# MAC-VO/MAC-VO

Measured on AMD Instinct MI355X. Metric: stereo frames/sec at 640x480 (hot path: cost volume + lookup, keypoint selection, covariance, PGO), higher is better.
Workload: dtype f32 via f16x2 (volume: fp32 operands row-scaled by powers of two and split into two fp16 pieces, three products, fp32 accumulate, scales undone exactly) + f32 (lookup/covariance) + f64 (PGO)

## Files before the change

mac-vo_amd/csrc/kp_select.hip:

```cpp
#include "common.h"
#include <math.h>

namespace {

#ifdef MV_KP_PROFILE
__device__ long long g_kp_stamps[16];
#define KP_STAMP(i) do { if (threadIdx.x == 0) g_kp_stamps[i] = wall_clock64(); } while (0)
#else
#define KP_STAMP(i)
#endif

constexpr int TILE_W = 64;
constexpr int TILE_H = 16;
constexpr int MAX_R = 7;
constexpr unsigned CAND_FLAG = 0x80000000u;

struct KpWs {
    unsigned long long* cand_bits;
    unsigned* rec_idx;
    float* rec_q;
    float* rec_d;
    int* counters;
    size_t lane_bytes;

    __device__ __forceinline__ KpWs lane(int l) const {
        const size_t o = (size_t)l * lane_bytes;
        return KpWs{(unsigned long long*)((char*)cand_bits + o), (unsigned*)((char*)rec_idx + o), (float*)((char*)rec_q + o),
                    (float*)((char*)rec_d + o), (int*)((char*)counters + o), lane_bytes};
    }
};

__device__ __forceinline__ float flow_quality(const float* __restrict__ fc, int plane, int idx) {
    const float c0 = fc[idx], c1 = fc[plane + idx], c2 = fc[2 * plane + idx];
    return (c0 + c1) - 2.f * c2;
}

__device__ __forceinline__ float nanmin(float a, float b) { return (a < b || a != a) ? a : b; }

template <bool FUSE>
__global__ __launch_bounds__(256) void kp_nms_kernel(const float* __restrict__ fc, const float* __restrict__ d0,
                                                      const float* __restrict__ d0c, const float* __restrict__ d1,
                                                      const float* __restrict__ d1c,
                                                      const uint8_t* __restrict__ mask_a,
                                                      const uint8_t* __restrict__ mask_b, mvKpSelectParams p,
                                                      KpWs ws_all, int words_per_row, mvEpiArgs ef) {
    MV_CHAIN_KERNEL_PRIO();
    const KpWs ws = ws_all.lane(blockIdx.z);
    {
        const size_t lp = (size_t)blockIdx.z * p.H * p.W;
        if (fc) fc += 3 * lp;
        if (d0) d0 += lp;
        if (d0c) d0c += lp;
        if (d1) d1 += lp;
        if (d1c) d1c += lp;
        if (mask_a) mask_a += lp;
        if (mask_b) mask_b += lp;
        if (FUSE) {
            ef.flow += 4 * lp; ef.logcov += 4 * lp;
            if (ef.disparity) ef.disparity += lp;
            if (ef.disparity_cov) ef.disparity_cov += lp;
            if (ef.depth) ef.depth += lp;
            if (ef.depth_cov) ef.depth_cov += lp;
            if (ef.bad_mask) ef.bad_mask += lp;
            if (ef.match_flow) ef.match_flow += 2 * lp;
            if (ef.match_cov) ef.match_cov += 3 * lp;
        }
    }
    __shared__ float tile[TILE_H + 2 * MAX_R][TILE_W + 2 * MAX_R + 1];
    __shared__ float hmin[TILE_H + 2 * MAX_R][TILE_W + 1];
    __shared__ int wg_count, wg_base;
    const int H = p.H, W = p.W, plane = H * W;
    const int r = p.kernel_size >> 1;
    const int x0 = blockIdx.x * TILE_W, y0 = blockIdx.y * TILE_H;
    const int tx = threadIdx.x, ty = threadIdx.y;
    const int tid = ty * 64 + tx;
    const bool mapping = p.mode == MV_KP_MAPPING;
    if (tid == 0) wg_count = 0;

    if (!mapping) {
        const int tw = TILE_W + 2 * r, th = TILE_H + 2 * r;
        constexpr int NST = ((TILE_W + 2 * MAX_R) * (TILE_H + 2 * MAX_R) + 255) / 256;
        float qv[NST];
#pragma unroll
        for (int i = 0; i < NST; ++i) {
            const int e = i * 256 + tid;
            const int ly = e / tw, lx = e - ly * tw;
            const int gx = x0 + lx - r, gy = y0 + ly - r;
            float q = INFINITY;
            if (e < tw * th && gx >= 0 && gx < W && gy >= 0 && gy < H) {
                const int idx = gy * W + gx;
                if (FUSE) {
                    const float l0 = ef.logcov[2 * plane + idx], l1 = ef.logcov[3 * plane + idx];
                    const float c0 = ef.cov_is_log ? expf(l0 * 2.f) : l0, c1 = ef.cov_is_log ? expf(l1 * 2.f) : l1;
                    q = (c0 + c1) - 2.f * 0.f;
                } else if (p.mode == MV_KP_NODEPTH) {
                    q = flow_quality(fc, plane, idx);
                } else {
                    q = d0c[idx] + d1c[idx];
                    if (fc) q = q * flow_quality(fc, plane, idx);
                }
            }
            qv[i] = q;
        }
#pragma unroll
        for (int i = 0; i < NST; ++i) {
            const int e = i * 256 + tid;
            const int ly = e / tw, lx = e - ly * tw;
            if (e < tw * th) tile[ly][lx] = qv[i];
        }
        __syncthreads();
        for (int e = tid; e < th * TILE_W; e += 256) {
            const int ly = e >> 6, lx = e & 63;
            float m = tile[ly][lx];
            for (int dx = 1; dx <= 2 * r; ++dx) m = nanmin(m, tile[ly][lx + dx]);
            hmin[ly][lx] = m;
        }
    }
    __syncthreads();

    bool nms_px[TILE_H / 4];
    bool cand_px[TILE_H / 4];
    float q_px[TILE_H / 4];
    int my_nms = 0;
#pragma unroll
    for (int it = 0; it < TILE_H / 4; ++it) {
        const int ly = ty * (TILE_H / 4) + it;
        const int gx = x0 + tx, gy = y0 + ly;
        const bool inimg = gx < W && gy < H;
        const int idx = gy * W + gx;
        bool nms = false, cand = false;
        float q = 0.f;
        if (FUSE && inimg) mv_epilogue_pixel(ef, plane, idx);
        if (inimg) {
            const bool border = p.mask_width > 0 && gx >= p.mask_width && gx < W - p.mask_width &&
                                gy >= p.mask_width && gy < H - p.mask_width;
            if (mapping) {
                cand = border && (d0[idx] < p.max_depth) && (d0c[idx] < p.max_depth_cov);
            } else {
                q = tile[ly + r][tx + r];
                float m = hmin[ly][tx];
                for (int dy = 1; dy <= 2 * r; ++dy) m = nanmin(m, hmin[ly + dy][tx]);
                nms = (q == m);
                cand = nms && border;
                if (cand && p.mode == MV_KP_FULL) cand = (d0[idx] < p.max_depth) && (d1[idx] < p.max_depth);
            }
            if (cand && mask_a) cand = mask_a[idx] != 0;
            if (cand && mask_b) cand = mask_b[idx] != 0;
        }
        const unsigned long long cand_word = __ballot(cand);
        if (tx == 0 && gy < H) ws.cand_bits[(size_t)gy * words_per_row + blockIdx.x] = cand_word;
        nms_px[it] = nms;
        cand_px[it] = cand;
        q_px[it] = q;
        my_nms += nms;
    }
    if (mapping) return;

    int my_off = 0;
    if (my_nms) my_off = atomicAdd(&wg_count, my_nms);
    __syncthreads();
#ifdef MV_KP_FAKE_ATOMIC
    if (tid == 0) wg_base = (blockIdx.y * gridDim.x + blockIdx.x) * 16;
#else
    if (tid == 0) wg_base = wg_count ? atomicAdd(&ws.counters[0], wg_count) : 0;
#endif
    __syncthreads();
    int pos = wg_base + my_off;
#pragma unroll
    for (int it = 0; it < TILE_H / 4; ++it) {
        if (nms_px[it]) {
            const int gx = x0 + tx, gy = y0 + ty * (TILE_H / 4) + it;
            const int idx = gy * W + gx;
            ws.rec_idx[pos] = (unsigned)(((gy * words_per_row + blockIdx.x) << 6) | tx) | (cand_px[it] ? CAND_FLAG : 0u);
            if (p.mode == MV_KP_NODEPTH) {
                ws.rec_q[pos] = q_px[it];
            } else {
                ws.rec_q[pos] = fc ? flow_quality(fc, plane, idx) : 0.f;
                ws.rec_d[pos] = d0c[idx];
            }
            ++pos;
        }
    }
}

__device__ __forceinline__ unsigned float_key(float f) {
    if (f != f) return 0xFFFFFFFFu;
    const unsigned u = __float_as_uint(f);
    return (u & 0x80000000u) ? ~u : (u | 0x80000000u);
}
__device__ __forceinline__ float key_float(unsigned k) {
    const unsigned u = (k & 0x80000000u) ? (k & 0x7FFFFFFFu) : ~k;
    return __uint_as_float(u);
}

#ifndef MV_KP_FINISH_THREADS
#define MV_KP_FINISH_THREADS 1024
#endif

constexpr int RANK_CAP = 256;
constexpr unsigned NAN_KEY = 0xFFFFFFFFu;

template <int NT>
__device__ __forceinline__ int block_exclusive_scan(int v, int* wave_tot , int& total) {
    constexpr int NW = NT / 64;
    const int tid = threadIdx.x;
    int incl = v;
#pragma unroll
    for (int o = 1; o < 64; o <<= 1) {
        const int t = __shfl_up(incl, o, 64);
        if ((tid & 63) >= o) incl += t;
    }
    __syncthreads();
    if ((tid & 63) == 63) wave_tot[tid >> 6] = incl;
    __syncthreads();
    int off = 0;
    total = 0;
#pragma unroll
    for (int w = 0; w < NW; ++w) {
        const int t = wave_tot[w];
        if (w < (tid >> 6)) off += t;
        total += t;
    }
    return off + incl - v;
}

template <int NT, bool CACHED, int RPT, typename F>
__device__ __forceinline__ void for_each_key(const float* __restrict__ vals, int n, const unsigned (&keys)[RPT], F&& f) {
    const int tid = threadIdx.x;
    if (CACHED) {
        const int nr = (n + NT - 1) / NT;
#pragma unroll
        for (int r = 0; r < RPT; ++r)
            if (r < nr && r * NT + tid < n) f(keys[r]);
    } else {
        for (int i = tid; i < n; i += NT) f(float_key(vals[i]));
    }
}

struct MedianLds {
    unsigned hist[2048];
    unsigned lst[RANK_CAP];
    unsigned red_lo[16], red_hi[16];
    int red_cnt[16];
    int wave_tot[16];
    int sh[4];
    unsigned res;
};

template <int NT, bool CACHED, int RPT>
__device__ float block_nanmedian(const float* __restrict__ vals, int n, const unsigned (&keys)[RPT], MedianLds& L) {
    constexpr int NW = NT / 64, BPT = 2048 / NT;
    const int tid = threadIdx.x;
    unsigned lo = NAN_KEY, hi = 0u;
    int cnt = 0;
    for_each_key<NT, CACHED, RPT>(vals, n, keys, [&](unsigned k) {
        if (k != NAN_KEY) {
            lo = min(lo, k);
            hi = max(hi, k);
            ++cnt;
        }
    });
#pragma unroll
    for (int o = 32; o > 0; o >>= 1) {
        lo = min(lo, (unsigned)__shfl_xor((int)lo, o, 64));
        hi = max(hi, (unsigned)__shfl_xor((int)hi, o, 64));
        cnt += __shfl_xor(cnt, o, 64);
    }
    __syncthreads();
    if ((tid & 63) == 0) {
        L.red_lo[tid >> 6] = lo;
        L.red_hi[tid >> 6] = hi;
        L.red_cnt[tid >> 6] = cnt;
    }
    __syncthreads();
    cnt = 0;
#pragma unroll
    for (int w = 0; w < NW; ++w) {
        lo = min(lo, L.red_lo[w]);
        hi = max(hi, L.red_hi[w]);
        cnt += L.red_cnt[w];
    }
    if (cnt <= 0) return NAN;
    int k = (cnt - 1) >> 1;
    for (;;) {
        if (lo == hi) return key_float(lo);
        const unsigned span = hi - lo;
        const int s = max(0, 32 - __clz((int)span) - 11);
#pragma unroll
        for (int j = 0; j < BPT; ++j) L.hist[j * NT + tid] = 0;
        if (tid == 0) L.sh[3] = 0;
        __syncthreads();
        for_each_key<NT, CACHED, RPT>(vals, n, keys, [&](unsigned kk) {
            if (kk >= lo && kk <= hi) atomicAdd(&L.hist[(kk - lo) >> s], 1u);
        });
        __syncthreads();
        int c[BPT], sum = 0;
#pragma unroll
        for (int j = 0; j < BPT; ++j) {
            c[j] = (int)L.hist[tid * BPT + j];
            sum += c[j];
        }
        int total;
        const int excl = block_exclusive_scan<NT>(sum, L.wave_tot, total);
        if (excl <= k && k < excl + sum) {
            int before = excl;
#pragma unroll
            for (int j = 0; j < BPT; ++j) {
                if (k >= before && k < before + c[j]) {
                    L.sh[0] = tid * BPT + j;
                    L.sh[1] = c[j];
                    L.sh[2] = k - before;
                }
                before += c[j];
            }
        }
        __syncthreads();
        const unsigned b = (unsigned)L.sh[0];
        const int cb = L.sh[1];
        k = L.sh[2];
        const unsigned nlo = lo + (b << s);
        const unsigned w = s ? ((1u << s) - 1u) : 0u;
        const unsigned nhi = (hi - nlo < w) ? hi : nlo + w;
        if (cb <= RANK_CAP) {
            for_each_key<NT, CACHED, RPT>(vals, n, keys, [&](unsigned kk) {
                if (kk >= nlo && kk <= nhi) L.lst[atomicAdd(&L.sh[3], 1)] = kk;
            });
            __syncthreads();
            for (int i = tid; i < cb; i += NT) {
                const unsigned e = L.lst[i];
                int rank = 0;
                for (int j = 0; j < cb; ++j) {
                    const unsigned o = L.lst[j];
                    rank += (o < e) || (o == e && j < i);
                }
                if (rank == k) L.res = e;
            }
            __syncthreads();
            return key_float(L.res);
        }
        lo = nlo;
        hi = nhi;
        __syncthreads();
    }
}

template <int NT, bool FAST, int RPT, int WPT, bool USE_D>
__device__ __forceinline__ void kp_finish_body(const mvKpSelectParams& p, const KpWs& ws, int has_flow, int words_per_row,
                                               int32_t* __restrict__ out_cand, int32_t* __restrict__ out_count,
                                               float* __restrict__ out_stats, int n_rec, MedianLds& L,
                                               unsigned long long* lds_words) {
    constexpr int RD = USE_D ? RPT : 1;
    const int tid = threadIdx.x;
    const int H = p.H, W = p.W;
    const bool mapping = p.mode == MV_KP_MAPPING;
    const bool use_f = (p.mode == MV_KP_NODEPTH) || (p.mode == MV_KP_FULL && has_flow);
    const bool use_d = USE_D && (p.mode == MV_KP_FULL);
    const int n_words = H * words_per_row;

    unsigned kq[RPT], kd[RD], ridx[RPT];
    unsigned long long wreg[WPT];
    KP_STAMP(0);
    if (FAST) {
        const int cap = H * W;
#pragma unroll
        for (int r = 0; r < RPT; ++r) {
            const int i = min(r * NT + tid, cap - 1);
            ridx[r] = mapping ? 0u : ws.rec_idx[i];
            kq[r] = use_f ? __float_as_uint(ws.rec_q[i]) : 0u;
            if (USE_D) kd[r] = use_d ? __float_as_uint(ws.rec_d[i]) : 0u;
        }
#pragma unroll
        for (int j = 0; j < WPT; ++j) {
            const int w = j * NT + tid;
            wreg[j] = w < n_words ? ws.cand_bits[w] : 0ull;
        }
#pragma unroll
        for (int r = 0; r < RPT; ++r) {
            const bool live = r * NT + tid < n_rec;
            ridx[r] = live ? ridx[r] : 0u;
            kq[r] = live ? float_key(__uint_as_float(kq[r])) : NAN_KEY;
            if (USE_D) kd[r] = live ? float_key(__uint_as_float(kd[r])) : NAN_KEY;
        }
    }

    float med_f = NAN, thr_f = INFINITY, med_d = NAN, thr_d = INFINITY;
    KP_STAMP(1);
    if (use_f) {
        med_f = block_nanmedian<NT, FAST, RPT>(ws.rec_q, n_rec, kq, L);
        const float prod = med_f * 1.5f;
        thr_f = (prod < p.max_match_cov) ? prod : p.max_match_cov;
    }
    if (use_d) {
        med_d = block_nanmedian<NT, FAST, RD>(ws.rec_d, n_rec, kd, L);
        const float prod = med_d * 1.5f;
        thr_d = (prod < p.max_depth_cov) ? prod : p.max_depth_cov;
    }

    KP_STAMP(2);
    const int per = (n_words + NT - 1) / NT;
    unsigned long long cw[WPT];
    if (FAST) {
        constexpr int NPASS = WPT > 5 * 1024 / NT ? 8 : 2;
        constexpr int TPP = NT / NPASS;
        unsigned fail = 0;
        if (!mapping) {
            const int nr = (n_rec + NT - 1) / NT;
#pragma unroll
            for (int r = 0; r < RPT; ++r) {
                if (r < nr && (ridx[r] & CAND_FLAG)) {
                    bool ok = true;
                    if (use_f) ok = key_float(kq[r]) < thr_f;
                    if (USE_D) { if (ok && use_d) ok = key_float(kd[USE_D ? r : 0]) < thr_d; }
                    if (!ok) fail |= 1u << r;
                }
            }
        }
#pragma unroll
        for (int i = 0; i < WPT; ++i) cw[i] = 0ull;
#pragma unroll 1
        for (int h = 0; h < NPASS; ++h) {
            const int wlo = h * TPP * per, whi = min(wlo + TPP * per, n_words);
#pragma unroll
            for (int j = 0; j < WPT; ++j) {
                const int w = j * NT + tid;
                if (w >= wlo && w < whi) lds_words[w - wlo] = wreg[j];
            }
            __syncthreads();
            if (fail) {
#pragma unroll
                for (int r = 0; r < RPT; ++r) {
                    const int w = (int)((ridx[r] & ~CAND_FLAG) >> 6);
                    if (((fail >> r) & 1u) && w >= wlo && w < whi) atomicAnd(&lds_words[w - wlo], ~(1ull << (ridx[r] & 63)));
                }
            }
            __syncthreads();
            if (tid / TPP == h) {
#pragma unroll
                for (int i = 0; i < WPT; ++i) {
                    const int w = tid * per + i;
                    if (i < per && w < whi) cw[i] = lds_words[w - wlo];
                }
            }
            __syncthreads();
        }
    } else if (!mapping) {
        for (int i = tid; i < n_rec; i += NT) {
            const unsigned ri = ws.rec_idx[i];
            if (ri & CAND_FLAG) {
                bool ok = true;
                if (use_f) ok = ws.rec_q[i] < thr_f;
                if (ok && use_d) ok = ws.rec_d[i] < thr_d;
                if (!ok) atomicAnd(&ws.cand_bits[(ri & ~CAND_FLAG) >> 6], ~(1ull << (ri & 63)));
            }
        }
        __threadfence();
        __syncthreads();
    }

    KP_STAMP(3);
    const int w_begin = min(tid * per, n_words), w_end = min(w_begin + per, n_words);
    int cnt = 0;
    if (FAST) {
#pragma unroll
        for (int i = 0; i < WPT; ++i) cnt += __popcll(cw[i]);
    } else {
        for (int w = w_begin; w < w_end; ++w)
            cnt += __popcll(__hip_atomic_load(&ws.cand_bits[w], __ATOMIC_RELAXED, __HIP_MEMORY_SCOPE_AGENT));
    }
    int total;
    int pos = block_exclusive_scan<NT>(cnt, L.wave_tot, total);
    KP_STAMP(4);
    auto emit = [&](unsigned long long bits, int w) {
        const int row = w / words_per_row, col0 = (w - row * words_per_row) * 64;
        while (bits) {
            const int bpos = __ffsll((long long)bits) - 1;
            bits &= bits - 1;
            out_cand[pos++] = row * W + col0 + bpos;
        }
    };
    if (FAST) {
#pragma unroll
        for (int i = 0; i < WPT; ++i)
            if (cw[i]) emit(cw[i], w_begin + i);
    } else {
        for (int w = w_begin; w < w_end; ++w)
            emit(__hip_atomic_load(&ws.cand_bits[w], __ATOMIC_RELAXED, __HIP_MEMORY_SCOPE_AGENT), w);
    }
    KP_STAMP(5);
    if (tid == 0) {
        ws.counters[0] = 0;
        out_count[0] = total;
        out_count[1] = n_rec;
        out_count[2] = 0;
        out_count[3] = 0;
        out_stats[0] = med_f;
        out_stats[1] = thr_f;
        out_stats[2] = med_d;
        out_stats[3] = thr_d;
    }
}

template <int NT, int RPT, int WPT, bool USE_D>
__global__ __launch_bounds__(NT) void kp_finish_kernel(mvKpSelectParams p, KpWs ws_all, int has_flow, int words_per_row,
                                                        int32_t* __restrict__ out_cand, int32_t* __restrict__ out_count,
                                                        float* __restrict__ out_stats) {
    __shared__ MedianLds L;
    extern __shared__ unsigned long long lds_words[];
    MV_CHAIN_KERNEL_PRIO();
    const KpWs ws = ws_all.lane(blockIdx.x);
    out_cand += (size_t)blockIdx.x * p.H * p.W;
    out_count += 4 * blockIdx.x;
    out_stats += 4 * blockIdx.x;
    const int n_rec = p.mode == MV_KP_MAPPING ? 0 : ws.counters[0];
    if (n_rec <= RPT * NT && p.H * words_per_row <= WPT * NT)
        kp_finish_body<NT, true, RPT, WPT, USE_D>(p, ws, has_flow, words_per_row, out_cand, out_count, out_stats, n_rec, L,
                                                  lds_words);
    else
        kp_finish_body<NT, false, RPT, WPT, USE_D>(p, ws, has_flow, words_per_row, out_cand, out_count, out_stats, n_rec, L,
                                                   lds_words);
}

template <int NT, int RPT, int WPT, bool USE_D>
static int launch_finish(const mvKpSelectParams& p, const KpWs& ws, int has_flow, int wpr, int32_t* out_cand,
                         int32_t* out_count, float* out_stats, int lanes, hipStream_t s) {
    const size_t dyn = (size_t)WPT * (NT / (WPT > 5 * 1024 / NT ? 8 : 2)) * sizeof(unsigned long long);
    hipLaunchKernelGGL((kp_finish_kernel<NT, RPT, WPT, USE_D>), dim3(lanes), dim3(NT), dyn, s, p, ws, has_flow, wpr, out_cand,
                       out_count, out_stats);
    return MV_OK;
}

__global__ __launch_bounds__(1024) void kp_map_scan_kernel(const unsigned long long* __restrict__ cand_bits, int n_words,
                                                            int* __restrict__ word_off, int32_t* __restrict__ out_count,
                                                            float* __restrict__ out_stats) {
    __shared__ int wave_tot[16];
    const int tid = threadIdx.x;
    const int per = (n_words + 1023) / 1024;
    const int w_begin = min(tid * per, n_words), w_end = min(w_begin + per, n_words);
    int cnt = 0;
    for (int w = w_begin; w < w_end; ++w) cnt += __popcll(cand_bits[w]);
    int total;
    int pos = block_exclusive_scan<1024>(cnt, wave_tot, total);
    for (int w = w_begin; w < w_end; ++w) {
        word_off[w] = pos;
        pos += __popcll(cand_bits[w]);
    }
    if (tid == 0) {
        out_count[0] = total;
        out_count[1] = out_count[2] = out_count[3] = 0;
        out_stats[0] = NAN;
        out_stats[1] = INFINITY;
        out_stats[2] = NAN;
        out_stats[3] = INFINITY;
    }
}

__global__ __launch_bounds__(256) void kp_map_emit_kernel(const unsigned long long* __restrict__ cand_bits,
                                                           const int* __restrict__ word_off, int n_words, int words_per_row,
                                                           int W, int32_t* __restrict__ out_cand) {
    const int w = blockIdx.x * 4 + (threadIdx.x >> 6);
    if (w >= n_words) return;
    const int lane = threadIdx.x & 63;
    const unsigned long long bits = cand_bits[w];
    if ((bits >> lane) & 1ull) {
        const int rank = __popcll(bits & ((1ull << lane) - 1ull));
        const int row = w / words_per_row, col0 = (w - row * words_per_row) * 64;
        out_cand[word_off[w] + rank] = row * W + col0 + lane;
    }
}

__global__ void kp_gather_kernel(const int32_t* __restrict__ cand, const int64_t* __restrict__ perm, mvLaneCounts cnt,
                                 int cap, size_t cand_lane_stride, int W, int64_t* __restrict__ out_uv) {
    const int i = blockIdx.x * blockDim.x + threadIdx.x;
    const int n_sel = cnt.n[blockIdx.y];
    cand += (size_t)blockIdx.y * cand_lane_stride;
    perm += (size_t)blockIdx.y * cap;
    out_uv += 2 * (size_t)blockIdx.y * cap;
    if (i < n_sel) {
        const int lin = cand[perm[i]];
        out_uv[2 * i + 0] = lin % W;
        out_uv[2 * i + 1] = lin / W;
    }
}

inline size_t align_up(size_t v, size_t a) { return (v + a - 1) / a * a; }

}

extern "C" size_t mv_kp_select_workspace_bytes(int H, int W) {
    if (H <= 0 || W <= 0) return 0;
    const size_t words = (size_t)H * mv_ceil_div(W, 64);
    return align_up(words * 8, 256) + 3 * align_up((size_t)H * W * 4, 256) + 256;
}

static int kp_select_impl(const float* flow_cov, const float* depth0, const float* depth0_cov, const float* depth1,
                          const float* depth1_cov, const uint8_t* mask_a, const uint8_t* mask_b, const mvKpSelectParams* params,
                          void* workspace, size_t workspace_bytes, int32_t* out_cand, int32_t* out_count, float* out_stats,
                          int lanes, mvStream_t stream, const mvEpiArgs* fuse) {
    MV_CHECK_ARG(lanes >= 1 && lanes <= MV_MAX_LANES);
    MV_CHECK_ARG(params && workspace && out_cand && out_count && out_stats);
    const mvKpSelectParams p = *params;
    MV_CHECK_ARG(p.H > 0 && p.W > 0 && p.mask_width >= 0);
    if (p.mode == MV_KP_NODEPTH) {
        MV_CHECK_ARG(flow_cov);
    } else if (p.mode == MV_KP_FULL) {
        MV_CHECK_ARG(depth0 && depth0_cov && depth1 && depth1_cov);
    } else if (p.mode == MV_KP_MAPPING) {
        MV_CHECK_ARG(depth0 && depth0_cov);
    } else {
        return MV_ERR_INVALID_ARG;
    }
    if (p.mode != MV_KP_MAPPING) {
        MV_CHECK_ARG(p.kernel_size >= 1 && (p.kernel_size & 1));
        if (p.kernel_size > 2 * MAX_R + 1) return MV_ERR_UNSUPPORTED;
    }
    const size_t lane_bytes = mv_kp_select_workspace_bytes(p.H, p.W);
    if (workspace_bytes < lane_bytes * (size_t)lanes) return MV_ERR_WORKSPACE;
    if (((uintptr_t)workspace & 7) != 0) return MV_ERR_INVALID_ARG;
    if (p.mode == MV_KP_MAPPING && lanes != 1) return MV_ERR_UNSUPPORTED;

    const int wpr = mv_ceil_div(p.W, 64);
    const size_t words = (size_t)p.H * wpr;
    const size_t plane_bytes = align_up((size_t)p.H * p.W * 4, 256);
    char* base = (char*)workspace;
    KpWs ws;
    ws.cand_bits = (unsigned long long*)base;
    base += align_up(words * 8, 256);
    ws.rec_idx = (unsigned*)base;
    base += plane_bytes;
    ws.rec_q = (float*)base;
    base += plane_bytes;
    ws.rec_d = (float*)base;
    base += plane_bytes;
    ws.counters = (int*)base;
    ws.lane_bytes = lane_bytes;

    hipStream_t s = (hipStream_t)stream;
    dim3 grid(wpr, mv_ceil_div(p.H, TILE_H), lanes), block(64, 4);
    if (fuse)
        hipLaunchKernelGGL(kp_nms_kernel<true>, grid, block, 0, s, flow_cov, depth0, depth0_cov, depth1, depth1_cov, mask_a,
                           mask_b, p, ws, wpr, *fuse);
    else
        hipLaunchKernelGGL(kp_nms_kernel<false>, grid, block, 0, s, flow_cov, depth0, depth0_cov, depth1, depth1_cov, mask_a,
                           mask_b, p, ws, wpr, mvEpiArgs{});
    if (p.mode == MV_KP_MAPPING) {
        const int n_words = p.H * wpr;
        int* word_off = (int*)ws.rec_idx;
        hipLaunchKernelGGL(kp_map_scan_kernel, dim3(1), dim3(1024), 0, s, ws.cand_bits, n_words, word_off, out_count, out_stats);
        hipLaunchKernelGGL(kp_map_emit_kernel, dim3(mv_ceil_div(n_words, 4)), dim3(256), 0, s, ws.cand_bits, word_off, n_words,
                           wpr, p.W, out_cand);
        return mv_launch_status();
    }
    const bool big = (size_t)p.H * wpr > 5 * (size_t)1024;
    const bool full = p.mode == MV_KP_FULL;
    int rc;
    static int small_nt = -1;
    if (small_nt < 0) { const char* e = getenv("MV_KP_FINISH_SMALL_NT"); small_nt = (e && atoi(e) == 512) ? 512 : 1024; }
    if (big) rc = full ? launch_finish<1024, 24, 15, true>(p, ws, flow_cov ? 1 : 0, wpr, out_cand, out_count, out_stats, lanes, s)
                       : launch_finish<1024, 24, 15, false>(p, ws, flow_cov ? 1 : 0, wpr, out_cand, out_count, out_stats, lanes, s);
    else if (small_nt == 512)
        rc = full ? launch_finish<512, 16, 10, true>(p, ws, flow_cov ? 1 : 0, wpr, out_cand, out_count, out_stats, lanes, s)
                  : launch_finish<512, 16, 10, false>(p, ws, flow_cov ? 1 : 0, wpr, out_cand, out_count, out_stats, lanes, s);
    else rc = full ? launch_finish<1024, 16, 5, true>(p, ws, flow_cov ? 1 : 0, wpr, out_cand, out_count, out_stats, lanes, s)
                   : launch_finish<1024, 16, 5, false>(p, ws, flow_cov ? 1 : 0, wpr, out_cand, out_count, out_stats, lanes, s);
    if (rc != MV_OK) return rc;
    return mv_launch_status();
}

extern "C" int mv_kp_select_lanes(const float* flow_cov, const float* depth0, const float* depth0_cov,
                                  const float* depth1, const float* depth1_cov, const uint8_t* mask_a,
                                  const uint8_t* mask_b, const mvKpSelectParams* params, void* workspace,
                                  size_t workspace_bytes, int32_t* out_cand, int32_t* out_count, float* out_stats,
                                  int lanes, mvStream_t stream) {
    return kp_select_impl(flow_cov, depth0, depth0_cov, depth1, depth1_cov, mask_a, mask_b, params, workspace, workspace_bytes,
                          out_cand, out_count, out_stats, lanes, stream, nullptr);
}

extern "C" int mv_frontend_epilogue_select_lanes(const float* flow, const float* logcov, int cov_is_log, float bl_fx,
                                                 float bl_fx_sq, float* disparity, float* disparity_cov, float* depth,
                                                 float* depth_cov, uint8_t* bad_mask, float* match_flow, float* match_cov,
                                                 const uint8_t* mask_a, const uint8_t* mask_b, const mvKpSelectParams* params,
                                                 void* workspace, size_t workspace_bytes, int32_t* out_cand,
                                                 int32_t* out_count, float* out_stats, int lanes, mvStream_t stream) {
    MV_CHECK_ARG(flow && logcov && params && match_cov);
    if (params->mode != MV_KP_NODEPTH) return MV_ERR_UNSUPPORTED;
    const mvEpiArgs ef{flow, logcov, cov_is_log, bl_fx, bl_fx_sq, disparity, disparity_cov, depth, depth_cov, match_flow, match_cov,
                       bad_mask};
    return kp_select_impl(match_cov, nullptr, nullptr, nullptr, nullptr, mask_a, mask_b, params, workspace, workspace_bytes,
                          out_cand, out_count, out_stats, lanes, stream, &ef);
}

extern "C" int mv_kp_select(const float* flow_cov, const float* depth0, const float* depth0_cov,
                            const float* depth1, const float* depth1_cov, const uint8_t* mask_a,
                            const uint8_t* mask_b, const mvKpSelectParams* params, void* workspace,
                            size_t workspace_bytes, int32_t* out_cand, int32_t* out_count, float* out_stats,
                            mvStream_t stream) {
    return mv_kp_select_lanes(flow_cov, depth0, depth0_cov, depth1, depth1_cov, mask_a, mask_b, params, workspace,
                              workspace_bytes, out_cand, out_count, out_stats, 1, stream);
}

extern "C" int mv_kp_gather_lanes(const int32_t* cand, size_t cand_lane_stride, const int64_t* perm, int lanes,
                                  const int32_t* n_live, int cap, int W, int64_t* out_uv, mvStream_t stream) {
    MV_CHECK_ARG(lanes >= 1 && lanes <= MV_MAX_LANES && n_live && cap >= 0 && W > 0);
    mvLaneCounts c{};
    int n_max = 0;
    for (int l = 0; l < lanes; ++l) {
        MV_CHECK_ARG(n_live[l] >= 0 && n_live[l] <= cap);
        c.n[l] = n_live[l];
        n_max = n_live[l] > n_max ? n_live[l] : n_max;
    }
    if (n_max == 0) return MV_OK;
    MV_CHECK_ARG(cand && perm && out_uv);
    hipLaunchKernelGGL(kp_gather_kernel, dim3(mv_ceil_div(n_max, 256), lanes), dim3(256), 0, (hipStream_t)stream, cand, perm,
                       c, cap, cand_lane_stride, W, out_uv);
    return mv_launch_status();
}

extern "C" int mv_kp_gather(const int32_t* cand, const int64_t* perm, int n_sel, int W, int64_t* out_uv,
                            mvStream_t stream) {
    MV_CHECK_ARG(n_sel >= 0);
    const int32_t n = n_sel;
    return mv_kp_gather_lanes(cand, 0, perm, 1, &n, n_sel, W, out_uv, stream);
}
```

Baseline: 7092.

## Write NMS keypoint records into fixed per-tile regions with overflow counter

The NMS kernel now gives each tile a fixed region of record slots, sized by the maximum number of NMS survivors for the kernel radius. Only tiles that exceed their cap take a global atomic for overflow slots, and unused slots are padded with NaN. The finish kernel reads the fixed region plus the overflow, derives liveness from NaN checks, and delays loading candidate words until after the flow median when depth is used, to lower register pressure. The aim is to cut global atomic contention and the serial wait on the counter, at the cost of a larger workspace and more records to scan in the finish kernel.

```diff
diff --git a/mac-vo_amd/csrc/kp_select.hip b/mac-vo_amd/csrc/kp_select.hip
--- a/mac-vo_amd/csrc/kp_select.hip
+++ b/mac-vo_amd/csrc/kp_select.hip
@@ -1,5 +1,7 @@
 #include "common.h"
 #include <math.h>
+#include <stdlib.h>
+#include <string.h>
 
 namespace {
 
@@ -14,6 +16,13 @@
 constexpr int TILE_H = 16;
 constexpr int MAX_R = 7;
 constexpr unsigned CAND_FLAG = 0x80000000u;
+constexpr int REGION_MIN_R = 3;
+constexpr int REGION_CAP_MAX = 64;
+
+__host__ __device__ inline int region_cap(int r) { return ((TILE_W + r) / (r + 1)) * ((TILE_H + r) / (r + 1)); }
+__host__ __device__ inline size_t record_slots(int H, int W) {
+    return (size_t)H * W + (size_t)((W + TILE_W - 1) / TILE_W) * ((H + TILE_H - 1) / TILE_H) * REGION_CAP_MAX;
+}
 
 struct KpWs {
     unsigned long long* cand_bits;
@@ -43,7 +52,7 @@
                                                       const float* __restrict__ d1c,
                                                       const uint8_t* __restrict__ mask_a,
                                                       const uint8_t* __restrict__ mask_b, mvKpSelectParams p,
-                                                      KpWs ws_all, int words_per_row, mvEpiArgs ef) {
+                                                      KpWs ws_all, int words_per_row, int reg_cap, mvEpiArgs ef) {
     MV_CHAIN_KERNEL_PRIO();
     const KpWs ws = ws_all.lane(blockIdx.z);
     {
@@ -159,6 +168,37 @@
     int my_off = 0;
     if (my_nms) my_off = atomicAdd(&wg_count, my_nms);
     __syncthreads();
+    if (reg_cap) {
+        const int n = wg_count;
+        const int region = (blockIdx.y * gridDim.x + blockIdx.x) * reg_cap;
+        if (n > reg_cap) {
+            if (tid == 0) wg_base = gridDim.x * gridDim.y * reg_cap + atomicAdd(&ws.counters[0], n - reg_cap);
+            __syncthreads();
+        }
+        int k = my_off;
+#pragma unroll
+        for (int it = 0; it < TILE_H / 4; ++it) {
+            if (nms_px[it]) {
+                const int gx = x0 + tx, gy = y0 + ty * (TILE_H / 4) + it;
+                const int idx = gy * W + gx;
+                const int pos = k < reg_cap ? region + k : wg_base + (k - reg_cap);
+                ws.rec_idx[pos] = (unsigned)(((gy * words_per_row + blockIdx.x) << 6) | tx) | (cand_px[it] ? CAND_FLAG : 0u);
+                if (p.mode == MV_KP_NODEPTH) {
+                    ws.rec_q[pos] = q_px[it];
+                } else {
+                    ws.rec_q[pos] = fc ? flow_quality(fc, plane, idx) : 0.f;
+                    ws.rec_d[pos] = d0c[idx];
+                }
+                ++k;
+            }
+        }
+        if (tid >= n && tid < reg_cap) {
+            ws.rec_idx[region + tid] = 0u;
+            ws.rec_q[region + tid] = NAN;
+            if (p.mode != MV_KP_NODEPTH) ws.rec_d[region + tid] = NAN;
+        }
+        return;
+    }
 #ifdef MV_KP_FAKE_ATOMIC
     if (tid == 0) wg_base = (blockIdx.y * gridDim.x + blockIdx.x) * 16;
 #else
@@ -243,6 +283,7 @@
     unsigned red_lo[16], red_hi[16];
     int red_cnt[16];
     int wave_tot[16];
+    int live_tot[16];
     int sh[4];
     unsigned res;
 };
@@ -344,10 +385,10 @@
     }
 }
 
-template <int NT, bool FAST, int RPT, int WPT, bool USE_D>
-__device__ __forceinline__ void kp_finish_body(const mvKpSelectParams& p, const KpWs& ws, int has_flow, int words_per_row,
+template <int NT, bool FAST, int RPT, int WPT, bool USE_D, bool REGION>
+__device__ __forceinline__ bool kp_finish_body(const mvKpSelectParams& p, const KpWs& ws, int has_flow, int words_per_row,
                                                int32_t* __restrict__ out_cand, int32_t* __restrict__ out_count,
-                                               float* __restrict__ out_stats, int n_rec, MedianLds& L,
+                                               float* __restrict__ out_stats, int n_rec, int reg_slots, MedianLds& L,
                                                unsigned long long* lds_words) {
     constexpr int RD = USE_D ? RPT : 1;
     const int tid = threadIdx.x;
@@ -357,31 +398,53 @@
     const bool use_d = USE_D && (p.mode == MV_KP_FULL);
     const int n_words = H * words_per_row;
 
+    constexpr bool DEFER_W = REGION && USE_D;
     unsigned kq[RPT], kd[RD], ridx[RPT];
     unsigned long long wreg[WPT];
     KP_STAMP(0);
+    int wave_live = 0;
     if (FAST) {
-        const int cap = H * W;
+        const int cap = REGION ? (int)record_slots(H, W) : H * W;
 #pragma unroll
         for (int r = 0; r < RPT; ++r) {
             const int i = min(r * NT + tid, cap - 1);
-            ridx[r] = mapping ? 0u : ws.rec_idx[i];
-            kq[r] = use_f ? __float_as_uint(ws.rec_q[i]) : 0u;
-            if (USE_D) kd[r] = use_d ? __float_as_uint(ws.rec_d[i]) : 0u;
-        }
-#pragma unroll
-        for (int j = 0; j < WPT; ++j) {
-            const int w = j * NT + tid;
-            wreg[j] = w < n_words ? ws.cand_bits[w] : 0ull;
+            ridx[r] = (mapping && !REGION) ? 0u : ws.rec_idx[i];
+            kq[r] = (use_f || REGION) ? __float_as_uint(ws.rec_q[i]) : 0u;
+            if (USE_D) kd[r] = (use_d || REGION) ? __float_as_uint(ws.rec_d[i]) : 0u;
+        }
+        if (!DEFER_W) {
+#pragma unroll
+            for (int j = 0; j < WPT; ++j) {
+                const int w = j * NT + tid;
+                wreg[j] = w < n_words ? ws.cand_bits[w] : 0ull;
+            }
+        }
+        if (REGION) {
+            const int n_ovf = ws.counters[0];
+            if (reg_slots + n_ovf > RPT * NT) return false;
+            n_rec = reg_slots + n_ovf;
         }
 #pragma unroll
         for (int r = 0; r < RPT; ++r) {
-            const bool live = r * NT + tid < n_rec;
+            const bool live = !REGION ? r * NT + tid < n_rec
+                                      : tid < reg_slots - r * NT ? !(__uint_as_float(kq[r]) != __uint_as_float(kq[r]))
+                                                                 : tid < n_rec - r * NT;
+            if (REGION) wave_live += __popcll(__ballot(live));
             ridx[r] = live ? ridx[r] : 0u;
             kq[r] = live ? float_key(__uint_as_float(kq[r])) : NAN_KEY;
             if (USE_D) kd[r] = live ? float_key(__uint_as_float(kd[r])) : NAN_KEY;
         }
     }
+
+    if (REGION && !FAST) {
+        n_rec = reg_slots + ws.counters[0];
+        for (int i0 = 0; i0 < n_rec; i0 += NT) {
+            const int i = i0 + tid;
+            const float q = i < n_rec ? ws.rec_q[i] : NAN;
+            wave_live += __popcll(__ballot(q == q));
+        }
+    }
+    if (REGION && (tid & 63) == 0) L.live_tot[tid >> 6] = wave_live;
 
     float med_f = NAN, thr_f = INFINITY, med_d = NAN, thr_d = INFINITY;
     KP_STAMP(1);
@@ -390,6 +453,12 @@
         const float prod = med_f * 1.5f;
         thr_f = (prod < p.max_match_cov) ? prod : p.max_match_cov;
     }
+    unsigned fail_f = 0;
+    if (DEFER_W && FAST && use_f) {
+#pragma unroll
+        for (int r = 0; r < RPT; ++r)
+            if ((ridx[r] & CAND_FLAG) && !(key_float(kq[r]) < thr_f)) fail_f |= 1u << r;
+    }
     if (use_d) {
         med_d = block_nanmedian<NT, FAST, RD>(ws.rec_d, n_rec, kd, L);
         const float prod = med_d * 1.5f;
@@ -400,6 +469,13 @@
     const int per = (n_words + NT - 1) / NT;
     unsigned long long cw[WPT];
     if (FAST) {
+        if (DEFER_W) {
+#pragma unroll
+            for (int j = 0; j < WPT; ++j) {
+                const int w = j * NT + tid;
+                wreg[j] = w < n_words ? ws.cand_bits[w] : 0ull;
+            }
+        }
         constexpr int NPASS = WPT > 5 * 1024 / NT ? 8 : 2;
         constexpr int TPP = NT / NPASS;
         unsigned fail = 0;
@@ -409,7 +485,8 @@
             for (int r = 0; r < RPT; ++r) {
                 if (r < nr && (ridx[r] & CAND_FLAG)) {
                     bool ok = true;
-                    if (use_f) ok = key_float(kq[r]) < thr_f;
+                    if (DEFER_W) ok = !((fail_f >> r) & 1u);
+                    else if (use_f) ok = key_float(kq[r]) < thr_f;
                     if (USE_D) { if (ok && use_d) ok = key_float(kd[USE_D ? r : 0]) < thr_d; }
                     if (!ok) fail |= 1u << r;
                 }
@@ -488,6 +565,11 @@
     }
     KP_STAMP(5);
     if (tid == 0) {
+        if (REGION) {
+            n_rec = 0;
+#pragma unroll
+            for (int w = 0; w < NT / 64; ++w) n_rec += L.live_tot[w];
+        }
         ws.counters[0] = 0;
         out_count[0] = total;
         out_count[1] = n_rec;
@@ -498,12 +580,13 @@
         out_stats[2] = med_d;
         out_stats[3] = thr_d;
     }
-}
-
-template <int NT, int RPT, int WPT, bool USE_D>
+    return true;
+}
+
+template <int NT, int RPT, int WPT, bool USE_D, bool REGION>
 __global__ __launch_bounds__(NT) void kp_finish_kernel(mvKpSelectParams p, KpWs ws_all, int has_flow, int words_per_row,
-                                                        int32_t* __restrict__ out_cand, int32_t* __restrict__ out_count,
-                                                        float* __restrict__ out_stats) {
+                                                        int reg_slots, int32_t* __restrict__ out_cand,
+                                                        int32_t* __restrict__ out_count, float* __restrict__ out_stats) {
     __shared__ MedianLds L;
     extern __shared__ unsigned long long lds_words[];
     MV_CHAIN_KERNEL_PRIO();
@@ -511,21 +594,30 @@
     out_cand += (size_t)blockIdx.x * p.H * p.W;
     out_count += 4 * blockIdx.x;
     out_stats += 4 * blockIdx.x;
+    if (REGION) {
+        if (reg_slots <= RPT * NT && p.H * words_per_row <= WPT * NT &&
+            kp_finish_body<NT, true, RPT, WPT, USE_D, true>(p, ws, has_flow, words_per_row, out_cand, out_count, out_stats, 0,
+                                                            reg_slots, L, lds_words))
+            return;
+        kp_finish_body<NT, false, RPT, WPT, USE_D, true>(p, ws, has_flow, words_per_row, out_cand, out_count, out_stats, 0,
+                                                         reg_slots, L, lds_words);
+        return;
+    }
     const int n_rec = p.mode == MV_KP_MAPPING ? 0 : ws.counters[0];
     if (n_rec <= RPT * NT && p.H * words_per_row <= WPT * NT)
-        kp_finish_body<NT, true, RPT, WPT, USE_D>(p, ws, has_flow, words_per_row, out_cand, out_count, out_stats, n_rec, L,
-                                                  lds_words);
+        kp_finish_body<NT, true, RPT, WPT, USE_D, false>(p, ws, has_flow, words_per_row, out_cand, out_count, out_stats, n_rec,
+                                                         0, L, lds_words);
     else
-        kp_finish_body<NT, false, RPT, WPT, USE_D>(p, ws, has_flow, words_per_row, out_cand, out_count, out_stats, n_rec, L,
-                                                   lds_words);
-}
-
-template <int NT, int RPT, int WPT, bool USE_D>
+        kp_finish_body<NT, false, RPT, WPT, USE_D, false>(p, ws, has_flow, words_per_row, out_cand, out_count, out_stats, n_rec,
+                                                          0, L, lds_words);
+}
+
+template <int NT, int RPT, int WPT, bool USE_D, bool REGION = false>
 static int launch_finish(const mvKpSelectParams& p, const KpWs& ws, int has_flow, int wpr, int32_t* out_cand,
-                         int32_t* out_count, float* out_stats, int lanes, hipStream_t s) {
+                         int32_t* out_count, float* out_stats, int lanes, hipStream_t s, int reg_slots = 0) {
     const size_t dyn = (size_t)WPT * (NT / (WPT > 5 * 1024 / NT ? 8 : 2)) * sizeof(unsigned long long);
-    hipLaunchKernelGGL((kp_finish_kernel<NT, RPT, WPT, USE_D>), dim3(lanes), dim3(NT), dyn, s, p, ws, has_flow, wpr, out_cand,
-                       out_count, out_stats);
+    hipLaunchKernelGGL((kp_finish_kernel<NT, RPT, WPT, USE_D, REGION>), dim3(lanes), dim3(NT), dyn, s, p, ws, has_flow, wpr,
+                       reg_slots, out_cand, out_count, out_stats);
     return MV_OK;
 }
 
@@ -589,7 +681,7 @@
 extern "C" size_t mv_kp_select_workspace_bytes(int H, int W) {
     if (H <= 0 || W <= 0) return 0;
     const size_t words = (size_t)H * mv_ceil_div(W, 64);
-    return align_up(words * 8, 256) + 3 * align_up((size_t)H * W * 4, 256) + 256;
+    return align_up(words * 8, 256) + 3 * align_up(record_slots(H, W) * 4, 256) + 256;
 }
 
 static int kp_select_impl(const float* flow_cov, const float* depth0, const float* depth0_cov, const float* depth1,
@@ -620,7 +712,7 @@
 
     const int wpr = mv_ceil_div(p.W, 64);
     const size_t words = (size_t)p.H * wpr;
-    const size_t plane_bytes = align_up((size_t)p.H * p.W * 4, 256);
+    const size_t plane_bytes = align_up(record_slots(p.H, p.W) * 4, 256);
     char* base = (char*)workspace;
     KpWs ws;
     ws.cand_bits = (unsigned long long*)base;
@@ -636,12 +728,25 @@
 
     hipStream_t s = (hipStream_t)stream;
     dim3 grid(wpr, mv_ceil_div(p.H, TILE_H), lanes), block(64, 4);
+    const bool big = (size_t)p.H * wpr > 5 * (size_t)1024;
+    static int small_nt = -1;
+    if (small_nt < 0) { const char* e = getenv("MV_KP_FINISH_SMALL_NT"); small_nt = (e && atoi(e) == 512) ? 512 : 1024; }
+    int reg_cap = 0, reg_slots = 0;
+    if (p.mode != MV_KP_MAPPING && (p.kernel_size >> 1) >= REGION_MIN_R && small_nt == 1024 && words <= 15 * (size_t)1024) {
+        const char* e = getenv("MV_KP_RECORDS");
+        const int cap = region_cap(p.kernel_size >> 1);
+        const size_t slots = (size_t)grid.x * grid.y * cap;
+        if (!(e && !strcmp(e, "counter")) && slots <= (size_t)(big ? 24 : 20) * 1024) {
+            reg_cap = cap;
+            reg_slots = (int)slots;
+        }
+    }
     if (fuse)
         hipLaunchKernelGGL(kp_nms_kernel<true>, grid, block, 0, s, flow_cov, depth0, depth0_cov, depth1, depth1_cov, mask_a,
-                           mask_b, p, ws, wpr, *fuse);
+                           mask_b, p, ws, wpr, reg_cap, *fuse);
     else
         hipLaunchKernelGGL(kp_nms_kernel<false>, grid, block, 0, s, flow_cov, depth0, depth0_cov, depth1, depth1_cov, mask_a,
-                           mask_b, p, ws, wpr, mvEpiArgs{});
+                           mask_b, p, ws, wpr, reg_cap, mvEpiArgs{});
     if (p.mode == MV_KP_MAPPING) {
         const int n_words = p.H * wpr;
         int* word_off = (int*)ws.rec_idx;
@@ -650,12 +755,16 @@
                            wpr, p.W, out_cand);
         return mv_launch_status();
     }
-    const bool big = (size_t)p.H * wpr > 5 * (size_t)1024;
     const bool full = p.mode == MV_KP_FULL;
+    const int hf = flow_cov ? 1 : 0;
     int rc;
-    static int small_nt = -1;
-    if (small_nt < 0) { const char* e = getenv("MV_KP_FINISH_SMALL_NT"); small_nt = (e && atoi(e) == 512) ? 512 : 1024; }
-    if (big) rc = full ? launch_finish<1024, 24, 15, true>(p, ws, flow_cov ? 1 : 0, wpr, out_cand, out_count, out_stats, lanes, s)
+    if (reg_cap && big)
+        rc = full ? launch_finish<1024, 24, 15, true, true>(p, ws, hf, wpr, out_cand, out_count, out_stats, lanes, s, reg_slots)
+                  : launch_finish<1024, 24, 15, false, true>(p, ws, hf, wpr, out_cand, out_count, out_stats, lanes, s, reg_slots);
+    else if (reg_cap)
+        rc = full ? launch_finish<1024, 20, 5, true, true>(p, ws, hf, wpr, out_cand, out_count, out_stats, lanes, s, reg_slots)
+                  : launch_finish<1024, 20, 5, false, true>(p, ws, hf, wpr, out_cand, out_count, out_stats, lanes, s, reg_slots);
+    else if (big) rc = full ? launch_finish<1024, 24, 15, true>(p, ws, flow_cov ? 1 : 0, wpr, out_cand, out_count, out_stats, lanes, s)
                        : launch_finish<1024, 24, 15, false>(p, ws, flow_cov ? 1 : 0, wpr, out_cand, out_count, out_stats, lanes, s);
     else if (small_nt == 512)
         rc = full ? launch_finish<512, 16, 10, true>(p, ws, flow_cov ? 1 : 0, wpr, out_cand, out_count, out_stats, lanes, s)
```

After: 7034. Within noise of the previous version (-0.8%).
